# jamesdolezal/biscuit

Measured on AMD Instinct MI355X. Metric: tiles/sec at MC-dropout=30, 299x299x3 (Xception, slide-level pred/sigma reduce), higher is better.
Workload: dtype f16; 1 GPU; BASELINE.json config 2: 1000 synthetic 299x299x3 tiles/slide, Xception f16 storage + MFMA, fp32 accumulation / BN / MC head, MC=30, batch=256, 17664 tiles/GPU resident in HBM; f16 is the 16-bit mode that holds the 1e-3 tile/slide tolerance on O(1)-logit weights (bf16, the type config 2 names, runs 5-6 % slower and misses it: bf16_value); mc_mode=head, mc_n=30, batch=256, hip_streams=1, grids_sized_for_mask=False, parallelism=slide-sharded dp1, one all-gather of slide (pred, sigma, n)

## Files before the change

biscuit_amd/csrc/kernels_front.hip:

```cpp
#include "gemm_common.h"

namespace {
using namespace bqk;

typedef float f32x2s __attribute__((ext_vector_type(2)));
typedef unsigned u32x4s __attribute__((ext_vector_type(4)));

constexpr int PX = 299, SO = 149, CO = 147;
constexpr int ROWB = PX * 3;
constexpr int NWF = 11;
constexpr int SW = 14;
constexpr float LO_SCALE = 1.0f / 2048.0f;

template <typename T>
struct FrontParams {
    const uint8_t* tiles;
    const unsigned long long* stats;
    const uint4* ws16;
    const float* s_scale;
    const float* s_bias;
    const uint4* wc16;
    const float* c_scale;
    const float* c_bias;
    T* out;
    int n, nstrips, nbands, items;
};

__device__ __forceinline__ void span(int s, int n, int ns, int& x0, int& nc) {
    const int base = n / ns, rem = n - base * ns;
    x0 = s * base + (s < rem ? s : rem);
    nc = base + (s < rem ? 1 : 0);
}

template <typename T> __device__ __forceinline__ f32x4 mmaT(const uint4& a, const uint4& b, const f32x4& c);
template <> __device__ __forceinline__ f32x4 mmaT<f16_t>(const uint4& a, const uint4& b, const f32x4& c) {
    return __builtin_amdgcn_mfma_f32_16x16x32_f16(__builtin_bit_cast(f16x8, a), __builtin_bit_cast(f16x8, b), c, 0, 0, 0);
}
template <> __device__ __forceinline__ f32x4 mmaT<bf16_t>(const uint4& a, const uint4& b, const f32x4& c) {
    return __builtin_amdgcn_mfma_f32_16x16x32_bf16(__builtin_bit_cast(bf16x8, a), __builtin_bit_cast(bf16x8, b), c, 0, 0, 0);
}

template <typename T> __device__ __forceinline__ _Float16 staged_f16(unsigned byte, float mean, float inv) {
    const float v = ((float)byte - mean) * inv;
    if constexpr (H16<T>::F16) return (_Float16)v;
    else return (_Float16)(float)(bf16_t)v;
}

template <typename T>
__global__ void __launch_bounds__(NWF * 64) front_stream_kernel(const FrontParams<T> p) {
    bq_f16_saturate();
    constexpr int NT = NWF * 64;
    constexpr int WS_BYTES = 2 * 2 * 1024;
    constexpr int WC_BYTES = 9 * 4 * 1024;
    constexpr int WC_OFF = WS_BYTES;
    constexpr int SB_OFF = WC_OFF + WC_BYTES;
    constexpr int PRIV_OFF = SB_OFF + 192 * 4;
    constexpr int U8_PITCH = 112;
    constexpr int U8_DW = 26;
    constexpr int PXP = 96;
    constexpr int RING_PITCH = 16 * PXP;
    constexpr int NRING = 4;
    constexpr int PRIV = 3 * U8_PITCH + NRING * RING_PITCH;
    extern __shared__ __attribute__((aligned(16))) unsigned char smem[];

    const int tid = threadIdx.x, lane = tid & 63;
    const int wave = __builtin_amdgcn_readfirstlane(tid >> 6);
    for (int i = tid; i < WS_BYTES / 16; i += NT) *reinterpret_cast<uint4*>(smem + i * 16) = p.ws16[i];
    for (int i = tid; i < WC_BYTES / 16; i += NT) *reinterpret_cast<uint4*>(smem + WC_OFF + i * 16) = p.wc16[i];
    if (tid < 32) {
        reinterpret_cast<float*>(smem + SB_OFF)[tid] = p.s_scale[tid];
        reinterpret_cast<float*>(smem + SB_OFF)[32 + tid] = p.s_bias[tid];
    }
    if (tid >= 64 && tid < 128) {
        reinterpret_cast<float*>(smem + SB_OFF)[64 + tid - 64] = p.c_scale[tid - 64];
        reinterpret_cast<float*>(smem + SB_OFF)[128 + tid - 64] = p.c_bias[tid - 64];
    }
    __syncthreads();

    unsigned char* const u8l = smem + PRIV_OFF + wave * PRIV;
    unsigned char* const ring = u8l + 3 * U8_PITCH;
    const int px = lane & 15, g = lane >> 4;
    const float* const sbs = reinterpret_cast<const float*>(smem + SB_OFF) + 8 * g;
    const float* const sbc = reinterpret_cast<const float*>(smem + SB_OFF) + 64 + 8 * g;
    int koff[8];
#pragma unroll
    for (int j = 0; j < 8; ++j) {
        const int k = 8 * g + j;
        koff[j] = k < 27 ? (k / 9) * U8_PITCH + (k % 9) : 0;
    }
    const int wgx = xcd_tile(blockIdx.x, gridDim.x);
    const __amdgpu_buffer_rsrc_t orsrc = __builtin_amdgcn_make_buffer_rsrc(
        p.out, 0, (int)((size_t)p.n * CO * CO * 64 * sizeof(T)), 0x00020000);

    for (int it = 0;; ++it) {
        const int item = __builtin_amdgcn_readfirstlane((it * (int)gridDim.x + wgx) * NWF + wave);
        if (item >= p.items) break;
        const int strip = item % p.nstrips;
        const int t1 = item / p.nstrips;
        const int band = t1 % p.nbands;
        const int img = t1 / p.nbands;
        int x0, nc, y0, nr;
        span(strip, CO, p.nstrips, x0, nc);
        span(band, CO, p.nbands, y0, nr);
        const int y1 = y0 + nr;
        float mean, inv;
        {
            const double nb = (double)(PX * PX * 3);
            const double mean_d = (double)p.stats[2 * img] / nb;
            double var = (double)p.stats[2 * img + 1] / nb - mean_d * mean_d;
            if (var < 0) var = 0;
            const double sd = sqrt(var), floor_sd = 1.0 / sqrt(nb);
            mean = (float)mean_d;
            inv = (float)(1.0 / (sd > floor_sd ? sd : floor_sd));
        }
        const long long tile_off = (long long)img * (PX * ROWB);
        const uintptr_t tb = reinterpret_cast<uintptr_t>(p.tiles);
        const long long last4 = (long long)p.n * (PX * ROWB) - 4;
        auto load_dw = [&](long long first_byte, int dw, int& shr_out, int& shl_out) -> unsigned {
            long long a4 = (long long)(((tb + (uintptr_t)first_byte) & ~(uintptr_t)3) - tb) + 4 * dw;
            const int shl = a4 < 0 ? (int)(-a4) * 8 : 0;
            long long over = a4 - last4;
            over = over < 0 ? 0 : (over > 3 ? 3 : over);
            a4 = a4 < 0 ? 0 : (a4 > last4 ? last4 : a4);
            shr_out = (int)over * 8;
            shl_out = shl;
            return *reinterpret_cast<const unsigned*>(p.tiles + a4);
        };
        const int lrow = lane >> 5, ldw = lane & 31;
        struct U8 { unsigned a, b; int a_r, a_l, b_r, b_l; };
        U8 uA{}, uB{};
        auto load_u8 = [&](int sy, U8& u) {
            const int syc = sy > SO - 1 ? SO - 1 : sy;
            const long long r0 = tile_off + (long long)(2 * syc) * ROWB + 6 * x0;
            u.a = load_dw(r0 + lrow * ROWB, ldw, u.a_r, u.a_l);
            u.b = load_dw(r0 + 2 * ROWB, ldw, u.b_r, u.b_l);
        };
        const uint8_t* const tile = p.tiles + tile_off;
        auto stem_row = [&](int sy, int slot, const U8& u) {
            const unsigned ua = u.a, ub = u.b;
            const int ua_r = u.a_r, ua_l = u.a_l, ub_r = u.b_r, ub_l = u.b_l;
            const int syc = sy > SO - 1 ? SO - 1 : sy;
            const uint8_t* r0 = tile + (size_t)(2 * syc) * ROWB + 6 * x0;
            const int sh0 = (int)(reinterpret_cast<uintptr_t>(r0) & 3), sh1 = (int)(reinterpret_cast<uintptr_t>(r0 + ROWB) & 3),
                      sh2 = (int)(reinterpret_cast<uintptr_t>(r0 + 2 * ROWB) & 3);
            {
                const int dwc = ldw < U8_DW ? ldw : U8_PITCH / 4 - 1;
                *reinterpret_cast<unsigned*>(u8l + lrow * U8_PITCH + 4 * dwc) = (ua >> ua_r) << ua_l;
                *reinterpret_cast<unsigned*>(u8l + 2 * U8_PITCH + 4 * dwc) = (ub >> ub_r) << ub_l;
            }
            {
                int s = px;
                if (x0 + s > SO - 1) s = SO - 1 - x0;
                _Float16 h[8];
#pragma unroll
                for (int j = 0; j < 8; ++j) {
                    const int k = 8 * g + j;
                    const int sh = k < 9 ? sh0 : (k < 18 ? sh1 : sh2);
                    const unsigned byte = u8l[koff[j] + sh + 6 * s];
                    h[j] = staged_f16<T>(byte, mean, inv);
                }
                uint4 b;
                b.x = __builtin_bit_cast(unsigned short, h[0]) | ((unsigned)__builtin_bit_cast(unsigned short, h[1]) << 16);
                b.y = __builtin_bit_cast(unsigned short, h[2]) | ((unsigned)__builtin_bit_cast(unsigned short, h[3]) << 16);
                b.z = __builtin_bit_cast(unsigned short, h[4]) | ((unsigned)__builtin_bit_cast(unsigned short, h[5]) << 16);
                b.w = __builtin_bit_cast(unsigned short, h[6]) | ((unsigned)__builtin_bit_cast(unsigned short, h[7]) << 16);
                f32x4 ah[2], al[2];
#pragma unroll
                for (int f = 0; f < 2; ++f) {
                    const uint4 wh = *reinterpret_cast<const uint4*>(smem + (f * 64 + lane) * 16);
                    const uint4 wl = *reinterpret_cast<const uint4*>(smem + ((2 + f) * 64 + lane) * 16);
                    ah[f] = mmaT<f16_t>(wh, b, (f32x4){0.f, 0.f, 0.f, 0.f});
                    al[f] = mmaT<f16_t>(wl, b, (f32x4){0.f, 0.f, 0.f, 0.f});
                }
                const float4 s0 = *reinterpret_cast<const float4*>(sbs), s1 = *reinterpret_cast<const float4*>(sbs + 4);
                const float4 c0 = *reinterpret_cast<const float4*>(sbs + 32), c1 = *reinterpret_cast<const float4*>(sbs + 36);
                float v[8];
#pragma unroll
                for (int i = 0; i < 4; ++i) {
                    v[i] = fmaf(al[0][i], LO_SCALE, ah[0][i]);
                    v[4 + i] = fmaf(al[1][i], LO_SCALE, ah[1][i]);
                }
                uint4 o;
                o.x = H16<T>::pack2(fmaxf(fmaf(v[0], s0.x, c0.x), 0.f), fmaxf(fmaf(v[1], s0.y, c0.y), 0.f));
                o.y = H16<T>::pack2(fmaxf(fmaf(v[2], s0.z, c0.z), 0.f), fmaxf(fmaf(v[3], s0.w, c0.w), 0.f));
                o.z = H16<T>::pack2(fmaxf(fmaf(v[4], s1.x, c1.x), 0.f), fmaxf(fmaf(v[5], s1.y, c1.y), 0.f));
                o.w = H16<T>::pack2(fmaxf(fmaf(v[6], s1.z, c1.z), 0.f), fmaxf(fmaf(v[7], s1.w, c1.w), 0.f));
                *reinterpret_cast<uint4*>(ring + slot * RING_PITCH + px * PXP + g * 16) = o;
            }
        };

        load_u8(y0, uA);
        load_u8(y0 + 1, uB);
        stem_row(y0, 0, uA);
        stem_row(y0 + 1, 1, uB);
        load_u8(y0 + 2, uA);
        load_u8(y0 + 3, uB);
#pragma unroll
        for (int q = 0; q < 4; ++q) __builtin_amdgcn_raw_buffer_store_b128((u32x4s){0u, 0u, 0u, 0u}, orsrc, (int)(0xffffff00u + 16 * q), 0, 0);
        int s0 = 0, s1 = 1, s2 = 2, s3 = 3;
        unsigned ooff = px < nc ? (unsigned)(((((size_t)img * CO + y0) * CO + x0 + px) * 64 + 8 * g) * sizeof(T)) : 0xffffff00u;
        const unsigned ostep = px < nc ? (unsigned)(CO * 64 * sizeof(T)) : 0u;
        for (int y = y0; y < y1; y += 2, ooff += 2 * ostep) {
            stem_row(y + 2, s2, uA);
            stem_row(y + 3, s3, uB);
            {
                const int last = y1 + 1;
                load_u8(y + 4 <= last ? y + 4 : last, uA);
                load_u8(y + 5 <= last ? y + 5 : last, uB);
            }
            __builtin_amdgcn_sched_barrier(0);
            f32x4 acc[2][4];
#pragma unroll
            for (int r = 0; r < 2; ++r)
#pragma unroll
                for (int f = 0; f < 4; ++f) acc[r][f] = (f32x4){0.f, 0.f, 0.f, 0.f};
            {
                uint4 b[4][3];
#pragma unroll
                for (int r = 0; r < 4; ++r) {
                    const int slot = r == 0 ? s0 : (r == 1 ? s1 : (r == 2 ? s2 : s3));
                    const unsigned char* rp = ring + slot * RING_PITCH + (px < SW ? px : SW - 1) * PXP + g * 16;
#pragma unroll
                    for (int dx = 0; dx < 3; ++dx) b[r][dx] = *reinterpret_cast<const uint4*>(rp + dx * PXP);
                }
                uint4 w[2][4];
                auto fetch = [&](int t, uint4 (&dst)[4]) {
#pragma unroll
                    for (int f = 0; f < 4; ++f) dst[f] = *reinterpret_cast<const uint4*>(smem + WC_OFF + ((t * 4 + f) * 64 + lane) * 16);
                };
                fetch(0, w[0]);
#pragma unroll
                for (int t = 0; t < 9; ++t) {
                    if (t + 1 < 9) fetch(t + 1, w[(t + 1) & 1]);
                    const int dy = t / 3, dx = t % 3;
#pragma unroll
                    for (int r = 0; r < 2; ++r)
#pragma unroll
                        for (int f = 0; f < 4; ++f) acc[r][f] = mmaT<T>(w[t & 1][f], b[dy + r][dx], acc[r][f]);
                }
            }
#pragma unroll
            for (int r = 0; r < 2; ++r) {
                const unsigned off = r == 0 ? ooff : (y + 1 < y1 ? ooff + ostep : 0xffffff00u);
#pragma unroll
                for (int q = 0; q < 2; ++q) {
                    const float4 a0 = *reinterpret_cast<const float4*>(sbc + 32 * q), a1 = *reinterpret_cast<const float4*>(sbc + 32 * q + 4);
                    const float4 b0 = *reinterpret_cast<const float4*>(sbc + 64 + 32 * q), b1 = *reinterpret_cast<const float4*>(sbc + 64 + 32 * q + 4);
                    const f32x4 u = acc[r][2 * q], v = acc[r][2 * q + 1];
                    u32x4s o;
                    o[0] = H16<T>::pack2(fmaxf(fmaf(u[0], a0.x, b0.x), 0.f), fmaxf(fmaf(u[1], a0.y, b0.y), 0.f));
                    o[1] = H16<T>::pack2(fmaxf(fmaf(u[2], a0.z, b0.z), 0.f), fmaxf(fmaf(u[3], a0.w, b0.w), 0.f));
                    o[2] = H16<T>::pack2(fmaxf(fmaf(v[0], a1.x, b1.x), 0.f), fmaxf(fmaf(v[1], a1.y, b1.y), 0.f));
                    o[3] = H16<T>::pack2(fmaxf(fmaf(v[2], a1.z, b1.z), 0.f), fmaxf(fmaf(v[3], a1.w, b1.w), 0.f));
                    __builtin_amdgcn_raw_buffer_store_b128(o, orsrc, (int)off + 64 * q, 0, 0);
                }
            }
            { const int t0 = s0, t1 = s1; s0 = s2; s1 = s3; s2 = t0; s3 = t1; }
        }
    }
}

template <typename T>
int launch_front_t(const uint8_t* tiles, const unsigned long long* stats, const void* ws16, const float* s_scale, const float* s_bias,
                   const void* wc16, const float* c_scale, const float* c_bias, void* out, int n, int num_cus, hipStream_t s) {
    FrontParams<T> p;
    p.tiles = tiles; p.stats = stats;
    p.ws16 = reinterpret_cast<const uint4*>(ws16); p.s_scale = s_scale; p.s_bias = s_bias;
    p.wc16 = reinterpret_cast<const uint4*>(wc16); p.c_scale = c_scale; p.c_bias = c_bias;
    p.out = reinterpret_cast<T*>(out);
    p.n = n;
    p.nstrips = (CO + SW - 1) / SW;
    const long long base_items = (long long)n * p.nstrips;
    const int waves = num_cus * NWF;
    int nb = (CO + 24) / 25;
    if (base_items * nb < waves) {
        nb = (int)((waves + base_items - 1) / base_items);
        if (nb > CO / 4) nb = CO / 4;
        if (nb < 1) nb = 1;
    }
    p.nbands = nb;
    p.items = (int)(base_items * nb);
    constexpr size_t lds = 2 * 2 * 1024 + 9 * 4 * 1024 + 192 * 4 + (size_t)NWF * (3 * 112 + 4 * 16 * 96);
    static_assert(lds <= 160 * 1024, "front kernel LDS budget");
    auto kern = front_stream_kernel<T>;
    static BqLdsAttr attr;
    if (const int e = attr.ensure(reinterpret_cast<const void*>(kern), lds)) return e;
    int grid = (p.items + NWF - 1) / NWF;
    if (grid > num_cus) grid = num_cus;
    hipLaunchKernelGGL(kern, dim3(grid), dim3(NWF * 64), lds, s, p);
    return (int)hipGetLastError();
}

}

int launch_front(int dtype, const uint8_t* tiles, const unsigned long long* stats, const void* ws16, const float* s_scale,
                 const float* s_bias, const void* wc16, const float* c_scale, const float* c_bias, void* out, int n, int num_cus,
                 hipStream_t s) {
    if (n <= 0) return 0;
    if (dtype == 0 || (long long)n * CO * CO * 64 * 2 > 0xffffff00ll) return (int)hipErrorInvalidValue;
    return dtype == 2 ? launch_front_t<f16_t>(tiles, stats, ws16, s_scale, s_bias, wc16, c_scale, c_bias, out, n, num_cus, s)
                      : launch_front_t<bf16_t>(tiles, stats, ws16, s_scale, s_bias, wc16, c_scale, c_bias, out, n, num_cus, s);
}
```

Baseline: 33710 tiles/s.

## Software-pipeline stem and conv stages in front kernel with six-slot ring

Restructures the fused stem+conv front kernel so each step interleaves the 3x3 conv MFMAs with the previous step's epilogue stores and the next rows' stem gather/convert/MFMA/BN. It uses sched_group_barrier hints and a six-slot ring with double-buffered u8 staging. BN scale/bias move into registers, address math drops to 32-bit with gather offsets precomputed, waves per block go from 11 to 8, and band count comes from a cost model. The aim is to hide LDS and global-load latency behind MFMA work. In exchange, register pressure rises, there are fewer waves per CU, and int32 address overflow becomes a risk for large n.

```diff
diff --git a/biscuit_amd/csrc/kernels_front.hip b/biscuit_amd/csrc/kernels_front.hip
--- a/biscuit_amd/csrc/kernels_front.hip
+++ b/biscuit_amd/csrc/kernels_front.hip
@@ -8,9 +8,27 @@
 
 constexpr int PX = 299, SO = 149, CO = 147;
 constexpr int ROWB = PX * 3;
-constexpr int NWF = 11;
+constexpr int NWF = 8;
 constexpr int SW = 14;
 constexpr float LO_SCALE = 1.0f / 2048.0f;
+constexpr int MIN_BAND = 4;
+constexpr int PROLOGUE_STEPS = 2;
+
+constexpr int WS_BYTES = 2 * 2 * 1024;
+constexpr int WC_BYTES = 9 * 4 * 1024;
+constexpr int WC_OFF = WS_BYTES;
+constexpr int SB_OFF = WC_OFF + WC_BYTES;
+constexpr int PRIV_OFF = SB_OFF + 192 * 4;
+constexpr int U8_PITCH = 112;
+constexpr int U8_DW = 26;
+constexpr int U8_STAGE = 3 * U8_PITCH;
+constexpr int PXP = 96;
+constexpr int RING_PITCH = 16 * PXP;
+constexpr int NRING = 6;
+constexpr int PRIV = 2 * U8_STAGE + NRING * RING_PITCH;
+constexpr size_t FRONT_LDS = PRIV_OFF + (size_t)NWF * PRIV;
+static_assert(FRONT_LDS <= 160 * 1024, "front kernel LDS budget");
+constexpr unsigned DROP = 0xffffff00u;
 
 template <typename T>
 struct FrontParams {
@@ -46,21 +64,21 @@
     else return (_Float16)(float)(bf16_t)v;
 }
 
+template <int NV, int NM = 8>
+__device__ __forceinline__ void mix() {
+#pragma unroll
+    for (int i = 0; i < NM; ++i) {
+        __builtin_amdgcn_sched_group_barrier(0x008, 1, 0);
+        __builtin_amdgcn_sched_group_barrier(0x002, NV, 0);
+        __builtin_amdgcn_sched_group_barrier(0x100, 1, 0);
+    }
+    __builtin_amdgcn_sched_barrier(0);
+}
+
 template <typename T>
 __global__ void __launch_bounds__(NWF * 64) front_stream_kernel(const FrontParams<T> p) {
     bq_f16_saturate();
     constexpr int NT = NWF * 64;
-    constexpr int WS_BYTES = 2 * 2 * 1024;
-    constexpr int WC_BYTES = 9 * 4 * 1024;
-    constexpr int WC_OFF = WS_BYTES;
-    constexpr int SB_OFF = WC_OFF + WC_BYTES;
-    constexpr int PRIV_OFF = SB_OFF + 192 * 4;
-    constexpr int U8_PITCH = 112;
-    constexpr int U8_DW = 26;
-    constexpr int PXP = 96;
-    constexpr int RING_PITCH = 16 * PXP;
-    constexpr int NRING = 4;
-    constexpr int PRIV = 3 * U8_PITCH + NRING * RING_PITCH;
     extern __shared__ __attribute__((aligned(16))) unsigned char smem[];
 
     const int tid = threadIdx.x, lane = tid & 63;
@@ -78,19 +96,34 @@
     __syncthreads();
 
     unsigned char* const u8l = smem + PRIV_OFF + wave * PRIV;
-    unsigned char* const ring = u8l + 3 * U8_PITCH;
+    unsigned char* const ring = u8l + 2 * U8_STAGE;
     const int px = lane & 15, g = lane >> 4;
-    const float* const sbs = reinterpret_cast<const float*>(smem + SB_OFF) + 8 * g;
-    const float* const sbc = reinterpret_cast<const float*>(smem + SB_OFF) + 64 + 8 * g;
-    int koff[8];
-#pragma unroll
-    for (int j = 0; j < 8; ++j) {
-        const int k = 8 * g + j;
-        koff[j] = k < 27 ? (k / 9) * U8_PITCH + (k % 9) : 0;
-    }
+    float sS[8], sB[8], cS[2][8], cB[2][8];
+    {
+        const float* const sbs = reinterpret_cast<const float*>(smem + SB_OFF) + 8 * g;
+        const float* const sbc = reinterpret_cast<const float*>(smem + SB_OFF) + 64 + 8 * g;
+#pragma unroll
+        for (int i = 0; i < 8; ++i) {
+            sS[i] = sbs[i];
+            sB[i] = sbs[32 + i];
+#pragma unroll
+            for (int q = 0; q < 2; ++q) {
+                cS[q][i] = sbc[32 * q + i];
+                cB[q][i] = sbc[64 + 32 * q + i];
+            }
+        }
+    }
+    const unsigned char* const rd = ring + (px < SW ? px : SW - 1) * PXP + g * 16;
+    unsigned char* const wr = ring + px * PXP + g * 16;
+    const int lrow = lane >> 5, ldw = lane & 31;
+    const int dwc = ldw < U8_DW ? ldw : U8_PITCH / 4 - 1;
+    unsigned char* const st_a = u8l + lrow * U8_PITCH + 4 * dwc;
+    unsigned char* const st_b = u8l + 2 * U8_PITCH + 4 * dwc;
     const int wgx = xcd_tile(blockIdx.x, gridDim.x);
     const __amdgpu_buffer_rsrc_t orsrc = __builtin_amdgcn_make_buffer_rsrc(
         p.out, 0, (int)((size_t)p.n * CO * CO * 64 * sizeof(T)), 0x00020000);
+    const int tbl = (int)(reinterpret_cast<uintptr_t>(p.tiles) & 3);
+    const int last4 = p.n * (PX * ROWB) - 4;
 
     for (int it = 0;; ++it) {
         const int item = __builtin_amdgcn_readfirstlane((it * (int)gridDim.x + wgx) * NWF + wave);
@@ -102,7 +135,7 @@
         int x0, nc, y0, nr;
         span(strip, CO, p.nstrips, x0, nc);
         span(band, CO, p.nbands, y0, nr);
-        const int y1 = y0 + nr;
+        const int y1 = y0 + nr, last = y1 + 1;
         float mean, inv;
         {
             const double nb = (double)(PX * PX * 3);
@@ -113,151 +146,229 @@
             mean = (float)mean_d;
             inv = (float)(1.0 / (sd > floor_sd ? sd : floor_sd));
         }
-        const long long tile_off = (long long)img * (PX * ROWB);
-        const uintptr_t tb = reinterpret_cast<uintptr_t>(p.tiles);
-        const long long last4 = (long long)p.n * (PX * ROWB) - 4;
-        auto load_dw = [&](long long first_byte, int dw, int& shr_out, int& shl_out) -> unsigned {
-            long long a4 = (long long)(((tb + (uintptr_t)first_byte) & ~(uintptr_t)3) - tb) + 4 * dw;
-            const int shl = a4 < 0 ? (int)(-a4) * 8 : 0;
-            long long over = a4 - last4;
-            over = over < 0 ? 0 : (over > 3 ? 3 : over);
-            a4 = a4 < 0 ? 0 : (a4 > last4 ? last4 : a4);
-            shr_out = (int)over * 8;
-            shl_out = shl;
-            return *reinterpret_cast<const unsigned*>(p.tiles + a4);
-        };
-        const int lrow = lane >> 5, ldw = lane & 31;
-        struct U8 { unsigned a, b; int a_r, a_l, b_r, b_l; };
-        U8 uA{}, uB{};
-        auto load_u8 = [&](int sy, U8& u) {
-            const int syc = sy > SO - 1 ? SO - 1 : sy;
-            const long long r0 = tile_off + (long long)(2 * syc) * ROWB + 6 * x0;
-            u.a = load_dw(r0 + lrow * ROWB, ldw, u.a_r, u.a_l);
-            u.b = load_dw(r0 + 2 * ROWB, ldw, u.b_r, u.b_l);
-        };
-        const uint8_t* const tile = p.tiles + tile_off;
-        auto stem_row = [&](int sy, int slot, const U8& u) {
-            const unsigned ua = u.a, ub = u.b;
-            const int ua_r = u.a_r, ua_l = u.a_l, ub_r = u.b_r, ub_l = u.b_l;
-            const int syc = sy > SO - 1 ? SO - 1 : sy;
-            const uint8_t* r0 = tile + (size_t)(2 * syc) * ROWB + 6 * x0;
-            const int sh0 = (int)(reinterpret_cast<uintptr_t>(r0) & 3), sh1 = (int)(reinterpret_cast<uintptr_t>(r0 + ROWB) & 3),
-                      sh2 = (int)(reinterpret_cast<uintptr_t>(r0 + 2 * ROWB) & 3);
+        const int fb0 = img * (PX * ROWB) + 2 * y0 * ROWB + 6 * x0;
+        const int shA = (tbl + fb0) & 3;
+        auto a4_of = [&](int sy, int rowsel) {
+            const int fb = fb0 + (2 * (sy - y0) + rowsel) * ROWB;
+            return fb - ((tbl + fb) & 3) + 4 * ldw;
+        };
+        struct U8 { unsigned a, b; int a_r, b_r; };
+        auto load_dw = [&](int a4, int& shr) -> unsigned {
+            const int c = a4 > last4 ? last4 : a4;
+            const int over = a4 - c;
+            shr = (over > 3 ? 3 : over) * 8;
+            return *reinterpret_cast<const unsigned*>(p.tiles + (unsigned)c);
+        };
+        auto load_u8 = [&](int a4a, int a4b, U8& u) {
+            u.a = load_dw(a4a, u.a_r);
+            u.b = load_dw(a4b, u.b_r);
+        };
+        auto stage_write = [&](int area, const U8& u, int shl_a) {
+            *reinterpret_cast<unsigned*>(st_a + area * U8_STAGE) = (u.a >> u.a_r) << shl_a;
+            *reinterpret_cast<unsigned*>(st_b + area * U8_STAGE) = u.b >> u.b_r;
+        };
+        int gA[8], gB[8];
+        {
+            int s = px;
+            if (x0 + s > SO - 1) s = SO - 1 - x0;
+#pragma unroll
+            for (int j = 0; j < 8; ++j) {
+                const int k = 8 * g + j;
+                const int kr = k < 27 ? k / 9 : 0, kb = k < 27 ? k - 9 * (k / 9) : 0;
+                gA[j] = kr * U8_PITCH + kb + 6 * s + ((shA + kr) & 3);
+                gB[j] = U8_STAGE + kr * U8_PITCH + kb + 6 * s + ((shA + 2 + kr) & 3);
+            }
+        }
+        auto gather = [&](const int (&ga)[8], unsigned (&by)[8]) {
+#pragma unroll
+            for (int j = 0; j < 8; ++j) by[j] = u8l[ga[j]];
+        };
+        auto convert = [&](const unsigned (&by)[8]) -> uint4 {
+            _Float16 h[8];
+#pragma unroll
+            for (int j = 0; j < 8; ++j) h[j] = staged_f16<T>(by[j], mean, inv);
+            uint4 b;
+            b.x = __builtin_bit_cast(unsigned short, h[0]) | ((unsigned)__builtin_bit_cast(unsigned short, h[1]) << 16);
+            b.y = __builtin_bit_cast(unsigned short, h[2]) | ((unsigned)__builtin_bit_cast(unsigned short, h[3]) << 16);
+            b.z = __builtin_bit_cast(unsigned short, h[4]) | ((unsigned)__builtin_bit_cast(unsigned short, h[5]) << 16);
+            b.w = __builtin_bit_cast(unsigned short, h[6]) | ((unsigned)__builtin_bit_cast(unsigned short, h[7]) << 16);
+            return b;
+        };
+        struct StemAcc { f32x4 ah[2], al[2]; };
+        struct StemW { uint4 h[2], l[2]; };
+        auto stem_weights = [&](StemW& w) {
+#pragma unroll
+            for (int f = 0; f < 2; ++f) {
+                w.h[f] = *reinterpret_cast<const uint4*>(smem + (f * 64 + lane) * 16);
+                w.l[f] = *reinterpret_cast<const uint4*>(smem + ((2 + f) * 64 + lane) * 16);
+            }
+        };
+        auto stem_mma = [&](const StemW& w, const uint4& b, StemAcc& a) {
+#pragma unroll
+            for (int f = 0; f < 2; ++f) {
+                a.ah[f] = mmaT<f16_t>(w.h[f], b, (f32x4){0.f, 0.f, 0.f, 0.f});
+                a.al[f] = mmaT<f16_t>(w.l[f], b, (f32x4){0.f, 0.f, 0.f, 0.f});
+            }
+        };
+        auto stem_bn = [&](const StemAcc& a, int slot) {
+            float v[8];
+#pragma unroll
+            for (int i = 0; i < 4; ++i) {
+                v[i] = fmaf(a.al[0][i], LO_SCALE, a.ah[0][i]);
+                v[4 + i] = fmaf(a.al[1][i], LO_SCALE, a.ah[1][i]);
+            }
+            uint4 o;
+            o.x = H16<T>::pack2(fmaxf(fmaf(v[0], sS[0], sB[0]), 0.f), fmaxf(fmaf(v[1], sS[1], sB[1]), 0.f));
+            o.y = H16<T>::pack2(fmaxf(fmaf(v[2], sS[2], sB[2]), 0.f), fmaxf(fmaf(v[3], sS[3], sB[3]), 0.f));
+            o.z = H16<T>::pack2(fmaxf(fmaf(v[4], sS[4], sB[4]), 0.f), fmaxf(fmaf(v[5], sS[5], sB[5]), 0.f));
+            o.w = H16<T>::pack2(fmaxf(fmaf(v[6], sS[6], sB[6]), 0.f), fmaxf(fmaf(v[7], sS[7], sB[7]), 0.f));
+            *reinterpret_cast<uint4*>(wr + slot * RING_PITCH) = o;
+        };
+        auto stem_row = [&](int area, int slot) {
+            unsigned by[8];
+            StemAcc a;
+            StemW w;
+            stem_weights(w);
+            gather(area == 0 ? gA : gB, by);
+            stem_mma(w, convert(by), a);
+            stem_bn(a, slot);
+        };
+        auto epilogue = [&](const f32x4& u, const f32x4& v, int q, unsigned off) {
+            u32x4s o;
+            o[0] = H16<T>::pack2(fmaxf(fmaf(u[0], cS[q][0], cB[q][0]), 0.f), fmaxf(fmaf(u[1], cS[q][1], cB[q][1]), 0.f));
+            o[1] = H16<T>::pack2(fmaxf(fmaf(u[2], cS[q][2], cB[q][2]), 0.f), fmaxf(fmaf(u[3], cS[q][3], cB[q][3]), 0.f));
+            o[2] = H16<T>::pack2(fmaxf(fmaf(v[0], cS[q][4], cB[q][4]), 0.f), fmaxf(fmaf(v[1], cS[q][5], cB[q][5]), 0.f));
+            o[3] = H16<T>::pack2(fmaxf(fmaf(v[2], cS[q][6], cB[q][6]), 0.f), fmaxf(fmaf(v[3], cS[q][7], cB[q][7]), 0.f));
+            __builtin_amdgcn_raw_buffer_store_b128(o, orsrc, (int)off + 64 * q, 0, 0);
+        };
+
+        U8 uA, uB;
+        int a4Aa = a4_of(y0, lrow), a4Ab = a4_of(y0, 2), a4Ba = a4_of(y0 + 1, lrow), a4Bb = a4_of(y0 + 1, 2);
+        {
+            const int shl = a4Aa < 0 ? -a4Aa * 8 : 0;
+            load_u8(a4Aa < 0 ? 0 : a4Aa, a4Ab, uA);
+            load_u8(a4Ba, a4Bb, uB);
+            U8 uC, uD;
+            load_u8(a4Aa + 4 * ROWB, a4Ab + 4 * ROWB, uC);
+            load_u8(a4Ba + 4 * ROWB, a4Bb + 4 * ROWB, uD);
+            stage_write(0, uA, shl);
+            stage_write(1, uB, 0);
+            stem_row(0, 0);
+            stem_row(1, 1);
+            stage_write(0, uC, 0);
+            stage_write(1, uD, 0);
+            stem_row(0, 2);
+            stem_row(1, 3);
+        }
+        a4Aa += 8 * ROWB; a4Ab += 8 * ROWB; a4Ba += 8 * ROWB; a4Bb += 8 * ROWB;
+        int rowA = y0 + 4, rowB = y0 + 5;
+        load_u8(a4Aa, a4Ab, uA);
+        load_u8(a4Ba, a4Bb, uB);
+#pragma unroll
+        for (int q = 0; q < 4; ++q) __builtin_amdgcn_raw_buffer_store_b128((u32x4s){0u, 0u, 0u, 0u}, orsrc, (int)(DROP + 16 * q), 0, 0);
+        unsigned ooff = px < nc ? (unsigned)(((((size_t)img * CO + y0) * CO + x0 + px) * 64 + 8 * g) * sizeof(T)) : DROP;
+        const unsigned ostep = px < nc ? (unsigned)(CO * 64 * sizeof(T)) : 0u;
+        f32x4 accP[2][4];
+#pragma unroll
+        for (int r = 0; r < 2; ++r)
+#pragma unroll
+            for (int f = 0; f < 4; ++f) accP[r][f] = (f32x4){0.f, 0.f, 0.f, 0.f};
+        unsigned offP0 = DROP, offP1 = DROP;
+        int y = y0;
+
+        auto step = [&](auto phase) {
+            constexpr int PH = decltype(phase)::value;
+            constexpr int S0 = (2 * PH) % NRING;
+            stage_write(0, uA, 0);
+            stage_write(1, uB, 0);
             {
-                const int dwc = ldw < U8_DW ? ldw : U8_PITCH / 4 - 1;
-                *reinterpret_cast<unsigned*>(u8l + lrow * U8_PITCH + 4 * dwc) = (ua >> ua_r) << ua_l;
-                *reinterpret_cast<unsigned*>(u8l + 2 * U8_PITCH + 4 * dwc) = (ub >> ub_r) << ub_l;
-            }
-            {
-                int s = px;
-                if (x0 + s > SO - 1) s = SO - 1 - x0;
-                _Float16 h[8];
-#pragma unroll
-                for (int j = 0; j < 8; ++j) {
-                    const int k = 8 * g + j;
-                    const int sh = k < 9 ? sh0 : (k < 18 ? sh1 : sh2);
-                    const unsigned byte = u8l[koff[j] + sh + 6 * s];
-                    h[j] = staged_f16<T>(byte, mean, inv);
-                }
-                uint4 b;
-                b.x = __builtin_bit_cast(unsigned short, h[0]) | ((unsigned)__builtin_bit_cast(unsigned short, h[1]) << 16);
-                b.y = __builtin_bit_cast(unsigned short, h[2]) | ((unsigned)__builtin_bit_cast(unsigned short, h[3]) << 16);
-                b.z = __builtin_bit_cast(unsigned short, h[4]) | ((unsigned)__builtin_bit_cast(unsigned short, h[5]) << 16);
-                b.w = __builtin_bit_cast(unsigned short, h[6]) | ((unsigned)__builtin_bit_cast(unsigned short, h[7]) << 16);
-                f32x4 ah[2], al[2];
-#pragma unroll
-                for (int f = 0; f < 2; ++f) {
-                    const uint4 wh = *reinterpret_cast<const uint4*>(smem + (f * 64 + lane) * 16);
-                    const uint4 wl = *reinterpret_cast<const uint4*>(smem + ((2 + f) * 64 + lane) * 16);
-                    ah[f] = mmaT<f16_t>(wh, b, (f32x4){0.f, 0.f, 0.f, 0.f});
-                    al[f] = mmaT<f16_t>(wl, b, (f32x4){0.f, 0.f, 0.f, 0.f});
-                }
-                const float4 s0 = *reinterpret_cast<const float4*>(sbs), s1 = *reinterpret_cast<const float4*>(sbs + 4);
-                const float4 c0 = *reinterpret_cast<const float4*>(sbs + 32), c1 = *reinterpret_cast<const float4*>(sbs + 36);
-                float v[8];
-#pragma unroll
-                for (int i = 0; i < 4; ++i) {
-                    v[i] = fmaf(al[0][i], LO_SCALE, ah[0][i]);
-                    v[4 + i] = fmaf(al[1][i], LO_SCALE, ah[1][i]);
-                }
-                uint4 o;
-                o.x = H16<T>::pack2(fmaxf(fmaf(v[0], s0.x, c0.x), 0.f), fmaxf(fmaf(v[1], s0.y, c0.y), 0.f));
-                o.y = H16<T>::pack2(fmaxf(fmaf(v[2], s0.z, c0.z), 0.f), fmaxf(fmaf(v[3], s0.w, c0.w), 0.f));
-                o.z = H16<T>::pack2(fmaxf(fmaf(v[4], s1.x, c1.x), 0.f), fmaxf(fmaf(v[5], s1.y, c1.y), 0.f));
-                o.w = H16<T>::pack2(fmaxf(fmaf(v[6], s1.z, c1.z), 0.f), fmaxf(fmaf(v[7], s1.w, c1.w), 0.f));
-                *reinterpret_cast<uint4*>(ring + slot * RING_PITCH + px * PXP + g * 16) = o;
-            }
-        };
-
-        load_u8(y0, uA);
-        load_u8(y0 + 1, uB);
-        stem_row(y0, 0, uA);
-        stem_row(y0 + 1, 1, uB);
-        load_u8(y0 + 2, uA);
-        load_u8(y0 + 3, uB);
-#pragma unroll
-        for (int q = 0; q < 4; ++q) __builtin_amdgcn_raw_buffer_store_b128((u32x4s){0u, 0u, 0u, 0u}, orsrc, (int)(0xffffff00u + 16 * q), 0, 0);
-        int s0 = 0, s1 = 1, s2 = 2, s3 = 3;
-        unsigned ooff = px < nc ? (unsigned)(((((size_t)img * CO + y0) * CO + x0 + px) * 64 + 8 * g) * sizeof(T)) : 0xffffff00u;
-        const unsigned ostep = px < nc ? (unsigned)(CO * 64 * sizeof(T)) : 0u;
-        for (int y = y0; y < y1; y += 2, ooff += 2 * ostep) {
-            stem_row(y + 2, s2, uA);
-            stem_row(y + 3, s3, uB);
-            {
-                const int last = y1 + 1;
-                load_u8(y + 4 <= last ? y + 4 : last, uA);
-                load_u8(y + 5 <= last ? y + 5 : last, uB);
-            }
+                const int dA = rowA + 2 <= last ? 4 * ROWB : 0, dB = rowB + 2 <= last ? 4 * ROWB : 0;
+                rowA += dA ? 2 : 0;
+                rowB += dB ? 2 : 0;
+                a4Aa += dA; a4Ab += dA; a4Ba += dB; a4Bb += dB;
+                load_u8(a4Aa, a4Ab, uA);
+                load_u8(a4Ba, a4Bb, uB);
+            }
+            uint4 b[4][3], w[2][4];
+            auto rows = [&](int r) {
+#pragma unroll
+                for (int dx = 0; dx < 3; ++dx) b[r][dx] = *reinterpret_cast<const uint4*>(rd + ((S0 + r) % NRING) * RING_PITCH + dx * PXP);
+            };
+            auto fetch = [&](int t) {
+#pragma unroll
+                for (int f = 0; f < 4; ++f) w[t & 1][f] = *reinterpret_cast<const uint4*>(smem + WC_OFF + ((t * 4 + f) * 64 + lane) * 16);
+            };
+            f32x4 acc[2][4];
+#pragma unroll
+            for (int r = 0; r < 2; ++r)
+#pragma unroll
+                for (int f = 0; f < 4; ++f) acc[r][f] = (f32x4){0.f, 0.f, 0.f, 0.f};
+            auto tap = [&](int t) {
+                const int dy = t / 3, dx = t % 3;
+#pragma unroll
+                for (int r = 0; r < 2; ++r)
+#pragma unroll
+                    for (int f = 0; f < 4; ++f) acc[r][f] = mmaT<T>(w[t & 1][f], b[dy + r][dx], acc[r][f]);
+            };
+            unsigned byA[8], byB[8];
+            uint4 op;
+            StemAcc sa;
+            StemW sw;
+            rows(0); rows(1); fetch(0);
             __builtin_amdgcn_sched_barrier(0);
-            f32x4 acc[2][4];
+            fetch(1); tap(0); epilogue(accP[0][0], accP[0][1], 0, offP0);
+            mix<3>();
+            fetch(2); rows(2); tap(1); epilogue(accP[0][2], accP[0][3], 1, offP0);
+            mix<3>();
+            fetch(3); tap(2); epilogue(accP[1][0], accP[1][1], 0, offP1);
+            mix<3>();
+            fetch(4); gather(gA, byA); tap(3); epilogue(accP[1][2], accP[1][3], 1, offP1);
+            mix<3>();
+            fetch(5); gather(gB, byB); stem_weights(sw); tap(4); op = convert(byA);
+            mix<5>();
+            fetch(6); tap(5); stem_mma(sw, op, sa); op = convert(byB);
+            mix<4, 12>();
+            fetch(7); rows(3); tap(6); stem_bn(sa, (S0 + 4) % NRING);
+            mix<4>();
+            fetch(8); tap(7); stem_mma(sw, op, sa);
+            mix<1, 12>();
+            tap(8); stem_bn(sa, (S0 + 5) % NRING);
+            mix<4>();
 #pragma unroll
             for (int r = 0; r < 2; ++r)
 #pragma unroll
-                for (int f = 0; f < 4; ++f) acc[r][f] = (f32x4){0.f, 0.f, 0.f, 0.f};
-            {
-                uint4 b[4][3];
-#pragma unroll
-                for (int r = 0; r < 4; ++r) {
-                    const int slot = r == 0 ? s0 : (r == 1 ? s1 : (r == 2 ? s2 : s3));
-                    const unsigned char* rp = ring + slot * RING_PITCH + (px < SW ? px : SW - 1) * PXP + g * 16;
-#pragma unroll
-                    for (int dx = 0; dx < 3; ++dx) b[r][dx] = *reinterpret_cast<const uint4*>(rp + dx * PXP);
-                }
-                uint4 w[2][4];
-                auto fetch = [&](int t, uint4 (&dst)[4]) {
-#pragma unroll
-                    for (int f = 0; f < 4; ++f) dst[f] = *reinterpret_cast<const uint4*>(smem + WC_OFF + ((t * 4 + f) * 64 + lane) * 16);
-                };
-                fetch(0, w[0]);
-#pragma unroll
-                for (int t = 0; t < 9; ++t) {
-                    if (t + 1 < 9) fetch(t + 1, w[(t + 1) & 1]);
-                    const int dy = t / 3, dx = t % 3;
-#pragma unroll
-                    for (int r = 0; r < 2; ++r)
-#pragma unroll
-                        for (int f = 0; f < 4; ++f) acc[r][f] = mmaT<T>(w[t & 1][f], b[dy + r][dx], acc[r][f]);
-                }
-            }
-#pragma unroll
-            for (int r = 0; r < 2; ++r) {
-                const unsigned off = r == 0 ? ooff : (y + 1 < y1 ? ooff + ostep : 0xffffff00u);
-#pragma unroll
-                for (int q = 0; q < 2; ++q) {
-                    const float4 a0 = *reinterpret_cast<const float4*>(sbc + 32 * q), a1 = *reinterpret_cast<const float4*>(sbc + 32 * q + 4);
-                    const float4 b0 = *reinterpret_cast<const float4*>(sbc + 64 + 32 * q), b1 = *reinterpret_cast<const float4*>(sbc + 64 + 32 * q + 4);
-                    const f32x4 u = acc[r][2 * q], v = acc[r][2 * q + 1];
-                    u32x4s o;
-                    o[0] = H16<T>::pack2(fmaxf(fmaf(u[0], a0.x, b0.x), 0.f), fmaxf(fmaf(u[1], a0.y, b0.y), 0.f));
-                    o[1] = H16<T>::pack2(fmaxf(fmaf(u[2], a0.z, b0.z), 0.f), fmaxf(fmaf(u[3], a0.w, b0.w), 0.f));
-                    o[2] = H16<T>::pack2(fmaxf(fmaf(v[0], a1.x, b1.x), 0.f), fmaxf(fmaf(v[1], a1.y, b1.y), 0.f));
-                    o[3] = H16<T>::pack2(fmaxf(fmaf(v[2], a1.z, b1.z), 0.f), fmaxf(fmaf(v[3], a1.w, b1.w), 0.f));
-                    __builtin_amdgcn_raw_buffer_store_b128(o, orsrc, (int)off + 64 * q, 0, 0);
-                }
-            }
-            { const int t0 = s0, t1 = s1; s0 = s2; s1 = s3; s2 = t0; s3 = t1; }
+                for (int f = 0; f < 4; ++f) accP[r][f] = acc[r][f];
+            offP0 = ooff;
+            offP1 = y + 1 < y1 ? ooff + ostep : DROP;
+            ooff += 2 * ostep;
+            y += 2;
+            __builtin_amdgcn_sched_barrier(0);
+        };
+        for (;;) {
+            step(std::integral_constant<int, 0>{});
+            if (y >= y1) break;
+            step(std::integral_constant<int, 1>{});
+            if (y >= y1) break;
+            step(std::integral_constant<int, 2>{});
+            if (y >= y1) break;
         }
-    }
+#pragma unroll
+        for (int r = 0; r < 2; ++r)
+#pragma unroll
+            for (int q = 0; q < 2; ++q) epilogue(accP[r][2 * q], accP[r][2 * q + 1], q, r == 0 ? offP0 : offP1);
+    }
+}
+
+inline int front_bands(long long base_items, int waves) {
+    int best = 1;
+    long long best_cost = -1;
+    for (int nb = 1; nb <= CO / MIN_BAND; ++nb) {
+        const int rows = (CO + nb - 1) / nb;
+        const long long rounds = (base_items * nb + waves - 1) / waves;
+        const long long cost = rounds * ((rows + 1) / 2 + PROLOGUE_STEPS);
+        if (best_cost < 0 || cost < best_cost) { best = nb; best_cost = cost; }
+    }
+    return best;
 }
 
 template <typename T>
@@ -271,23 +382,14 @@
     p.n = n;
     p.nstrips = (CO + SW - 1) / SW;
     const long long base_items = (long long)n * p.nstrips;
-    const int waves = num_cus * NWF;
-    int nb = (CO + 24) / 25;
-    if (base_items * nb < waves) {
-        nb = (int)((waves + base_items - 1) / base_items);
-        if (nb > CO / 4) nb = CO / 4;
-        if (nb < 1) nb = 1;
-    }
-    p.nbands = nb;
-    p.items = (int)(base_items * nb);
-    constexpr size_t lds = 2 * 2 * 1024 + 9 * 4 * 1024 + 192 * 4 + (size_t)NWF * (3 * 112 + 4 * 16 * 96);
-    static_assert(lds <= 160 * 1024, "front kernel LDS budget");
+    p.nbands = front_bands(base_items, (num_cus > 0 ? num_cus : 1) * NWF);
+    p.items = (int)(base_items * p.nbands);
     auto kern = front_stream_kernel<T>;
     static BqLdsAttr attr;
-    if (const int e = attr.ensure(reinterpret_cast<const void*>(kern), lds)) return e;
+    if (const int e = attr.ensure(reinterpret_cast<const void*>(kern), FRONT_LDS)) return e;
     int grid = (p.items + NWF - 1) / NWF;
     if (grid > num_cus) grid = num_cus;
-    hipLaunchKernelGGL(kern, dim3(grid), dim3(NWF * 64), lds, s, p);
+    hipLaunchKernelGGL(kern, dim3(grid), dim3(NWF * 64), FRONT_LDS, s, p);
     return (int)hipGetLastError();
 }
 
```

Measured after the change: 33810 tiles/s (median of 4 runs). About the same (+0.3%).
